# DARYL-GWZ/Proud-SLAM

Measured on AMD Instinct MI355X. Metric: rays/sec render+backward, Replica room0, 64 samples/ray, 1/2/4/8 MI355X, higher is better.
Workload: dtype f32

## Files before the change

### include/psvo.h

```cpp
#ifndef PSVO_H
#define PSVO_H

#include <stdint.h>

#ifdef __cplusplus
extern "C" {
#endif

enum {
    PSVO_OK = 0,
    PSVO_E_INVALID = 1,
    PSVO_E_LAUNCH = 2,
    PSVO_E_OVERFLOW = 3,
    PSVO_E_BUSY = 4,
    PSVO_E_SYSTEM = 5
};

const char *psvo_last_error(void);
const char *psvo_version(void);


int psvo_svo_intersect(void *stream, int b, int n, int m, float voxelsize, int n_max, const float *ray_start,
                       const float *ray_dir, const float *points, const int *children, int *idx, float *min_depth,
                       float *max_depth);
// ... 216 lines not shown

typedef struct psvo_pixel_frame {
    const float *dirs;
    const float *rgb;
    const float *depth;
    uint8_t *mask;
} psvo_pixel_frame;
int64_t psvo_sample_pixels_workspace_ints(int n_frames, int64_t n_pix);
int psvo_sample_pixels(void *stream, int n_frames, int64_t n_pix, int64_t k, const float *weights, int joint_sum,
                       const float *u, uint64_t seed, const psvo_pixel_frame *frames, int *workspace, int64_t *idx,
                       float *out_dirs, float *out_rgb, float *out_depth);

int64_t psvo_rows_workspace_ints(int64_t n_rows);
int psvo_rows_compact(void *stream, int64_t n_rows, int width, const float *grad, int *workspace, int *ids,
                      float *rows, int *count);
int psvo_rows_scatter_add(void *stream, int64_t n_list, int width, const int *ids, const float *rows, float *grad);
int psvo_rows_compact_flagged(void *stream, int64_t n_rows, int width, const float *grad, const uint8_t *flags,
                              int *workspace, int *ids, float *rows, int *count);
int psvo_rows_clear(void *stream, int64_t n_list, int width, const int *ids, float *grad, uint8_t *flags);
int psvo_rows_mark(void *stream, int64_t n_list, const int *ids, uint8_t *flags);
int psvo_rows_flags_from_grad(void *stream, int64_t n_rows, int width, const float *grad, uint8_t *flags);

psvo_engine *psvo_engine_new(void);
void psvo_engine_free(psvo_engine *e);
enum { PSVO_XCH_GATHER_I32 = 1, PSVO_XCH_SUM_I32 = 2, PSVO_XCH_SUM_F64 = 3, PSVO_XCH_QUERY = 0x100 };
typedef int (*psvo_exchange_fn)(void *user, int op, int64_t in_off, int64_t out_off, int64_t count, void *stream);
int64_t psvo_engine_exchange_words(int world, int64_t max_rays_global, int64_t max_rays_rank);
int psvo_engine_set_exchange(psvo_engine *e, int rank, int world, int64_t max_rays_global, int64_t max_rays_rank,
                             psvo_exchange_fn fn, void *user, int *xi32, double *xf64);

int psvo_engine_queued(psvo_engine *e);
int psvo_map_discard(psvo_engine *e);

enum { PSVO_PATH_QUERY_SPLIT = 1, PSVO_PATH_PADDED = 2, PSVO_PATH_DENSE_DECODER = 4 };
int psvo_engine_set_paths(psvo_engine *e, int paths);

int psvo_engine_select_stats(psvo_engine *e, void *stream, int64_t *out, int reset);

int psvo_engine_gate_stream(psvo_engine *e, void *stream);

int psvo_debug_set_lookback(int mask, int spin_bound, int delay_us);
int psvo_debug_lb_helps(int64_t *out3, int reset);
int psvo_debug_set_pixel_draw(int mode);
int psvo_debug_select_samples(void *stream, int64_t r_hit, int s_max, float truncation, float max_depth,
                              const int *offsets, const int *ray_ns, const float *z_vals, int z_stride,
                              const int *rank_ray, const float *gt_depth, const float *sdf_s, const float *feat,
                              const int *leaf, const float *t, const int *ray_of, int64_t cap, int split, int *cidx,
                              int *offa, int *offb, float *feat_c, int *leaf_c, float *t_c, int *ray_of_c,
                              float *rgb_c, int *src_c, int *counts, uint64_t *desc, uint32_t tag, int *host_flag);
int64_t psvo_debug_select_granules(int64_t r_hit);
int psvo_debug_composite_loss(void *stream, int64_t r_hit, int s_max, float truncation, float max_depth,
                              const int *offsets, const int *ray_ns, const float *z_vals, int z_stride,
                              const int *rank_ray, const float *gt_rgb, const float *gt_depth, const float *sdf_s,
                              const float *rgb_s, const float *coef, float *workspace, float *color, float *depth,
                              float *grad_sdf_s, float *grad_rgb_s, int partials, const int *cidx);

enum { PSVO_TIME_MLP_FWD = 0, PSVO_TIME_MLP_BWD = 1, PSVO_TIME_INTERP_FWD = 2, PSVO_TIME_INTERP_BWD = 3,
       PSVO_TIME_INTERSECT = 4, PSVO_TIME_SAMPLE = 5, PSVO_TIME_POINTS = 6, PSVO_TIME_SELECT = 7,
       PSVO_TIME_REGIONS = 8 };
int psvo_engine_set_timing(psvo_engine *e, int on);
int psvo_engine_timing(psvo_engine *e, double *mean_ms);
int psvo_engine_set_clock(psvo_engine *e, int max_steps);
int psvo_engine_clock(psvo_engine *e, double *period_ms, int *n_steps);
int psvo_host_wait_stats(double *wait_us, long long *calls, long long *waited, int reset);

int psvo_map_query(psvo_engine *e, void *stream, const psvo_map_desc *d, int64_t n_rays, const float *rays_o,
                   const float *rays_d, uint64_t seed);
int psvo_map_step(psvo_engine *e, void *stream, const psvo_map_desc *d, int64_t n_rays, const float *rays_o,
                  const float *rays_d, const float *gt_rgb, const float *gt_depth, uint64_t seed, int64_t adam_step,
                  int flags, float *loss_out, int *stats_out);

typedef struct psvo_map_frames {
    int n_frames;
    int64_t rays_per_frame;
    const float *dirs_cam;
    float *poses, *pose_m, *pose_v;
    const int64_t *pose_step;
    double lr_pose;
    float *pose_grad;
    const float *next_dirs_cam;
    uint64_t next_seed;
    void *next_stream;
    const float *next_gt_depth;
// ... 105 lines not shown
```

### proud-slam_amd/csrc/engine.cpp

```cpp
#include <stdio.h>
#include <stdlib.h>
#include <string.h>

#include <utility>

#include "engine_internal.h"

namespace psvo {
RenderWs *&engine_render_ws(psvo_engine *e) { return e->render; }
bool engine_data_parallel(const psvo_engine *e) { return e->x.on(); }
}

using namespace psvo;
using namespace psvo::eng;

namespace psvo {
thread_local KernelClock *g_kclock = nullptr;

namespace eng {

void *arena_buf(Arena &a, hipStream_t st, int slot, size_t bytes, int *rc) {
    if (bytes == 0) bytes = 16;
    if (a.cap[slot] >= bytes) return a.p[slot];
    if (a.p[slot]) {
// ... 189 lines not shown
    for (int i = 0; i < cnt; ++i) steps[i] = adam_step;
    for (int f = 0; pa && f < pa->n; ++f, ++cnt) {
        p[cnt] = pa->p[f];
        g[cnt] = pa->g[f];
        m[cnt] = pa->m[f];
        v[cnt] = pa->v[f];
        n[cnt] = 6;
        lr[cnt] = pa->lr;
        zero[cnt] = 0;
        steps[cnt] = pa->step[f];
    }
    return adam_launch(st, cnt, p, g, m, v, n, lr, d->beta1, d->beta2, d->eps, 0.0, adam_step, zero, steps, rows);
}

int pose_adam(hipStream_t st, const psvo_map_desc *d, const PoseAdam &pa) {
    if (pa.n == 0) return PSVO_OK;
    int64_t n6[kXchMaxFrames];
    double lr[kXchMaxFrames];
    int zero[kXchMaxFrames];
    for (int k = 0; k < pa.n; ++k) {
        n6[k] = 6;
        lr[k] = pa.lr;
        zero[k] = 0;
    }
    return adam_launch(st, pa.n, pa.p, pa.g, pa.m, pa.v, n6, lr, d->beta1, d->beta2, d->eps, 0.0, 1, zero,
                       const_cast<int64_t *>(pa.step));
}

}
}

extern "C" psvo_engine *psvo_engine_new(void) {
    psvo_engine *e = new psvo_engine();
    for (auto &q : e->qs)
        if (query_set_init(q) != PSVO_OK) {
            psvo_engine_free(e);
            return nullptr;
        }
    return e;
}

static EngineExchange exchange_layout(int world, int64_t max_rays_global, int64_t max_rays_rank) {
    EngineExchange x;
    x.world = world;
    x.nch = dist_slot0_rows(max_rays_global) / kSamplerG;
    x.max_rays_rank = max_rays_rank > 0 ? max_rays_rank : max_rays_global;
    x.cw = dist_count_words((int)x.max_rays_rank);
    return x;
}

extern "C" int64_t psvo_engine_exchange_words(int world, int64_t max_rays_global, int64_t max_rays_rank) {
    if (world < 1 || max_rays_global < 1 || max_rays_rank < 0 || max_rays_rank > max_rays_global) return -1;
    const EngineExchange x = exchange_layout(world, max_rays_global, max_rays_rank);
    return x.table_off() + x.table_words();
}

extern "C" int psvo_engine_set_exchange(psvo_engine *e, int rank, int world, int64_t max_rays_global,
                                        int64_t max_rays_rank, psvo_exchange_fn fn, void *user, int *xi32,
                                        double *xf64) {
    PSVO_REQUIRE(e, "engine_set_exchange: null engine");
    PSVO_REQUIRE(world >= 1 && rank >= 0 && rank < world && max_rays_global >= 1 && max_rays_rank >= 0 &&
                     max_rays_rank <= max_rays_global,
                 "engine_set_exchange: bad rank %d / world %d / max_rays_global %lld / max_rays_rank %lld", rank,
                 world, (long long)max_rays_global, (long long)max_rays_rank);
    PSVO_REQUIRE(e->q_count == 0, "engine_set_exchange: queries are queued");
    PSVO_REQUIRE(!fn || (xi32 && xf64), "engine_set_exchange: exchange buffers required");
    e->x = exchange_layout(world, max_rays_global, max_rays_rank);
    e->x.fn = fn;
    e->x.user = user;
    e->x.rank = rank;
    e->x.xi32 = xi32;
    e->x.xf64 = xf64;
    return PSVO_OK;
}

extern "C" int psvo_engine_set_paths(psvo_engine *e, int paths) {
    PSVO_REQUIRE(e && (paths & ~(PSVO_PATH_QUERY_SPLIT | PSVO_PATH_PADDED | PSVO_PATH_DENSE_DECODER)) == 0, "engine_set_paths: bad arguments");
    PSVO_REQUIRE(e->q_count == 0, "engine_set_paths: queries are queued");
    e->paths = paths;
    return PSVO_OK;
}

extern "C" int psvo_engine_gate_stream(psvo_engine *e, void *stream) {
    PSVO_REQUIRE(e, "engine_gate_stream: null engine");
    e->draw_gate_used = true;
    if (!e->draw_gate_recorded) return PSVO_OK;
    return st_wait(as_stream(stream), e->draw_gate_ev, "engine_gate_stream");
}

extern "C" int psvo_engine_select_stats(psvo_engine *e, void *stream, int64_t *out, int reset) {
    PSVO_REQUIRE(e && out, "engine_select_stats: null argument");
    for (int i = 0; i < 5; ++i) out[i] = 0;
    if (!e->a.p[kSelCnt]) return PSVO_OK;
    hipStream_t st = as_stream(stream);
    int c[psvo::kSelCountInts];
    if (hipMemcpyAsync(c, e->a.p[kSelCnt], sizeof(c), hipMemcpyDeviceToHost, st) != hipSuccess ||
        hipStreamSynchronize(st) != hipSuccess)
        return set_error(PSVO_E_LAUNCH, "engine_select_stats: copy failed");
    unsigned long long u[3];
    memcpy(u, c + 4, sizeof(u));
    out[0] = (int64_t)c[0] + c[1];
    out[1] = c[3];
    out[2] = (int64_t)u[0];
    out[3] = (int64_t)u[1];
    out[4] = (int64_t)u[2];
    if (c[2] & psvo::kLbFlagTimeout) {
        ENG_CALL(zero_async(static_cast<int *>(e->a.p[kSelCnt]) + 2, sizeof(int), st, "engine_select_stats"));
        if (e->host_flags) *(volatile int *)e->host_flags = 0;
        e->sel_zero_gen = 0;
        return set_error(PSVO_E_LAUNCH, "engine_select_stats: a sample selection's look-back wait was abandoned");
// ... 163 lines not shown
```

### proud-slam_amd/csrc/engine_step.cpp

```cpp
#include <stdint.h>
#include <string.h>

#include <algorithm>

#include "engine_internal.h"

using namespace psvo;
using namespace psvo::eng;

namespace {

struct Samples {
    int *offsets = nullptr, *leaf = nullptr, *ray_of = nullptr;
    float *tt = nullptr, *feat = nullptr, *rgb_s = nullptr, *act = nullptr;
    uint64_t *masks = nullptr;
};

struct Render {
    int64_t r_hit = 0, m = 0;
    int s_max = 0;
    int *rank_ray = nullptr, *ray_rank = nullptr, *ray_ns = nullptr;
    float *z_vals = nullptr, *images = nullptr, *sdf_s = nullptr;
    Samples s;
    float *sdf = nullptr, *weights = nullptr, *color = nullptr, *depth = nullptr;
    bool z_recorded = false;
    int z_stride = 0;
    bool sparse = false;
    float *h2 = nullptr;
};

constexpr int64_t kW128 = 128;
constexpr int kCritFlags = PSVO_CRIT_USE_COLOR | PSVO_CRIT_USE_DEPTH | PSVO_CRIT_USE_SDF;

void render_begin(QuerySet &qset, const Readback &rb, Render &o) {
    o.r_hit = rb.r_hit;
    o.m = rb.m;
    o.s_max = rb.s_max;
    o.rank_ray = static_cast<int *>(qset.a.p[kRankRay]);
// ... 98 lines not shown
        ENG_CALL(fork_join(st, e->aux, e->prep_fork));
        ENG_CALL(mlp_images(e->aux, c.d->width, c.d->dec, images));
        ENG_CALL(ev_record(e->prep_done, e->aux, c.who));
    }
    return PSVO_OK;
}

struct EarlyFwd {
    bool on = false;
    int64_t cap = 0;
    float *feat = nullptr, *sdf = nullptr, *h2 = nullptr;
};
int device_forward(const MapRender &c, const Images &im, Render &o, EarlyFwd &ef) {
    psvo_engine *e = c.e;
    hipStream_t st = c.st;
    const psvo_map_desc *d = c.d;
    QuerySet &qset = c.qset;
    int rc = PSVO_OK;
    const int64_t m_early = std::min<int64_t>(e->m_early, (int64_t)qset.R * qset.max_steps);
    ef.on = c.rays_path && c.sparse && qset.compacted && qset.a.p[kMDev] && m_early > 0 && im.ready() &&
            !(e->paths & PSVO_PATH_QUERY_SPLIT);
    if (!ef.on) return PSVO_OK;
    ef.cap = m_early;
    const int *m_dev = static_cast<const int *>(qset.a.p[kMDev]);
    ENG_BUF(float, fe, kFeat, m_early * 16 * sizeof(float));
    ENG_BUF(float, se, kSdfS, m_early * sizeof(float));
    ef.feat = fe;
    ef.sdf = se;
    if (d->width == 128) {
        ENG_BUF(float, he, kH2, m_early * kW128 * sizeof(float));
        ef.h2 = he;
    }
    ENG_CALL(join_adam(e, st, c.who, 2000.0));
    mark(e, st, PSVO_TIME_INTERP_FWD, 0);
    ENG_CALL(psvo::interp_fwd_dev(st, m_early, m_dev, d->voxel_size, static_cast<const int *>(qset.a.p[kLeafQ]),
                                  static_cast<const float *>(qset.a.p[kTQ]),
                                  static_cast<const int *>(qset.a.p[kRayOfQ]),
                                  static_cast<const int *>(qset.a.p[kRankRay]), c.rays_o, c.rays_d, d->centres,
                                  d->vertex_idx, d->emb, ef.feat));
    mark(e, st, PSVO_TIME_INTERP_FWD, 1);
    mark(e, st, PSVO_TIME_MLP_FWD, 0);
    if (im.on_aux) ENG_CALL(st_wait(st, e->prep_done, c.who));
    const psvo::H2Rows h2o{ef.h2, nullptr, nullptr};
    ENG_CALL(mlp_fwd_prepared(st, m_early, d->width, ef.feat, im.buf, ef.sdf, nullptr, nullptr, nullptr, m_dev, &h2o));
    if (engine_overlap(e) && c.need_z_event) {
        ENG_CALL(ev_record(e->z_ready, st, c.who));
        o.z_recorded = true;
    }
    return PSVO_OK;
}

int place_samples(const MapRender &c, Render &o) {
    psvo_engine *e = c.e;
    hipStream_t st = c.st;
    QuerySet &qset = c.qset;
    if (!c.rays_path) {
        ENG_CALL(padded_samples(e, st, qset, o));
        if (engine_overlap(e)) {
            ENG_CALL(ev_record(e->z_ready, st, c.who));
            o.z_recorded = true;
        }
        return PSVO_OK;
    }
    if (qset.compacted) {
        o.s.leaf = static_cast<int *>(qset.a.p[kLeafQ]);
        o.s.tt = static_cast<float *>(qset.a.p[kTQ]);
        o.s.ray_of = static_cast<int *>(qset.a.p[kRayOfQ]);
    }
    if (engine_overlap(e) && c.need_z_event && !o.z_recorded) {
        ENG_CALL(ev_record(e->z_ready, st, c.who));
        o.z_recorded = true;
    }
    if (!qset.compacted) {
        mark(e, st, PSVO_TIME_POINTS, 0);
        ENG_CALL(psvo::compact_rays(st, o.r_hit, qset.max_steps, static_cast<const int *>(qset.a.p[kSIdx]),
                                    static_cast<const float *>(qset.a.p[kSDepth]), o.s.offsets, o.s.leaf, o.s.tt,
                                    o.s.ray_of));
// ... 639 lines not shown
```

### proud-slam_amd/csrc/interp_load.h

```cpp
#pragma once

#include "psvo_common.h"

namespace psvo {

struct InterpSrc {
    const int *leaf, *ray_of, *ray_index, *vertex_idx;
    const float *t, *rays_o, *rays_d, *centres;
    const float4 *emb;
    float voxel_size;
};

int mlp_fwd_interp(hipStream_t st, int64_t m_cap, const int *m_dev, const InterpSrc &ip, const float *images,
                   float *sdf, float *rgb);

namespace iload {

__device__ __forceinline__ void load_x_interp(const InterpSrc &ip, int64_t s, bool valid, int h, float (&x)[8]) {
    float f[8];
#pragma unroll
    for (int i = 0; i < 8; ++i) f[i] = 0.0f;
    if (valid) {
        const int lf = ip.leaf[s];
        const int r = ip.ray_index[ip.ray_of[s]];
        const float ts = ip.t[s];
        float p[3];
#pragma unroll
        for (int a = 0; a < 3; ++a) {
            const float xa = __fadd_rn(ip.rays_o[(int64_t)r * 3 + a], __fmul_rn(ip.rays_d[(int64_t)r * 3 + a], ts));
            p[a] = __fadd_rn(__fdiv_rn(__fsub_rn(xa, ip.centres[(int64_t)lf * 3 + a]), ip.voxel_size), 0.5f);
        }
        const float ax[2] = {__fsub_rn(1.0f, p[0]), p[0]};
        const float ay[2] = {__fsub_rn(1.0f, p[1]), p[1]};
        const float az[2] = {__fsub_rn(1.0f, p[2]), p[2]};
        const int4 v0 = *reinterpret_cast<const int4 *>(ip.vertex_idx + (int64_t)lf * 8);
        const int4 v1 = *reinterpret_cast<const int4 *>(ip.vertex_idx + (int64_t)lf * 8 + 4);
        const int vid[8] = {v0.x, v0.y, v0.z, v0.w, v1.x, v1.y, v1.z, v1.w};
        float4 e0[8], e1[8];
#pragma unroll
        for (int k = 0; k < 8; ++k) {
            e0[k] = ip.emb[(int64_t)vid[k] * 4 + 2 * h];
            e1[k] = ip.emb[(int64_t)vid[k] * 4 + 2 * h + 1];
        }
#pragma unroll
        for (int k = 0; k < 8; ++k) {
            const float w = __fmul_rn(__fmul_rn(ax[(k >> 2) & 1], ay[(k >> 1) & 1]), az[k & 1]);
            f[0] = __fadd_rn(f[0], __fmul_rn(w, e0[k].x));
            f[1] = __fadd_rn(f[1], __fmul_rn(w, e0[k].y));
            f[2] = __fadd_rn(f[2], __fmul_rn(w, e0[k].z));
            f[3] = __fadd_rn(f[3], __fmul_rn(w, e0[k].w));
            f[4] = __fadd_rn(f[4], __fmul_rn(w, e1[k].x));
            f[5] = __fadd_rn(f[5], __fmul_rn(w, e1[k].y));
            f[6] = __fadd_rn(f[6], __fmul_rn(w, e1[k].z));
            f[7] = __fadd_rn(f[7], __fmul_rn(w, e1[k].w));
        }
    }
#pragma unroll
    for (int j = 0; j < 4; ++j) {
        const float send = h ? f[2 * j] : f[2 * j + 1];
        const float recv = __shfl_xor(send, 32, 64);
        x[j] = h ? recv : f[2 * j];
        x[4 + j] = h ? f[2 * j + 1] : recv;
    }
}

}
}
```

### proud-slam_amd/csrc/mlp.hip

```cpp
#include <hip/hip_runtime.h>

#include <cstdlib>

#include "interp_fuse.h"
#include "interp_load.h"
#include "psvo_common.h"

#ifdef PSVO_STAMPS
__device__ unsigned long long psvo_g_stamps[3][256][8][8][16];
#endif

namespace psvo {
namespace {

typedef float f32x16 __attribute__((ext_vector_type(16)));

constexpr int kW = 128;
constexpr int kIn = 16;
constexpr int kNB = kW / 32;

constexpr int kOffB1 = 0, kOffB2 = kOffB1 + 128, kOffB3 = kOffB2 + 128, kOffB4 = kOffB3 + 132,
              kOffB5 = kOffB4 + 128;
constexpr int kOffW3r0 = kOffB5 + 4, kOffW5 = kOffW3r0 + 128;
constexpr int kOffW = kOffW5 + 3 * 128;
// ... 644 lines not shown
                    const_cast<float *>(cm), 0, __builtin_amdgcn_readfirstlane((int)tbytes), 0x00020000);
#pragma unroll
                for (int r = 0; r < 16; ++r)
                    __builtin_amdgcn_raw_buffer_store_b32(__float_as_uint(bacc[3][r]), rc,
                                                          cfs.voff[((r >> 1) & 1) + 2 * ((r >> 2) & 1)],
                                                          4096 * 3 + 1024 * (r >> 2) + 128 * (r & 3), 0);
            }
        }
        ++seq;
        const uint64_t m4 = (uint64_t)half4[0] | ((uint64_t)half4[1] << 32);
        if (save_mask && valid) {
            uint64_t *mk = masks + (s * 2 + h) * 3;
            mk[0] = m1;
            mk[1] = m2;
            mk[2] = m4;
        }
        float rgb[3];
#pragma unroll
        for (int c = 0; c < 3; ++c) rgb[c] = sigmoidf(lds[kOffB5 + c] + row_dot(lds + kOffW5 + 128 * c, bacc, h));
        if (valid && h == 0) {
            sdf_out[s] = sdf;
            rgb_out[s * 3 + 0] = rgb[0];
            rgb_out[s * 3 + 1] = rgb[1];
            rgb_out[s * 3 + 2] = rgb[2];
        }
        if (!H2) PSVO_STAMP(8);
        PSVO_STAMP_FLUSH(0);
    }
    wait_vm(0);
}

constexpr int kLdsSdf2 = (kF2Buf0 + 16384) * 4;

template <bool IP = false>
__global__ __launch_bounds__(kF2Threads, 1) void k_mlp_sdf2(int64_t m_host, const float *__restrict__ feat,
                                                            const float *__restrict__ img,
                                                            float *__restrict__ sdf_out, const int *__restrict__ m_dev,
                                                            float *__restrict__ h2_out, InterpSrc ip) {
    extern __shared__ __attribute__((aligned(16))) float lds[];
    int64_t m = m_dev ? (int64_t)__builtin_amdgcn_readfirstlane(*m_dev) : m_host;
    if (m > m_host) m = 0;
    const int lane = threadIdx.x & 63;
    const int wave = threadIdx.x >> 6;
    const int h = lane >> 5;
    float *w2 = lds + kF2Buf0;
    const int64_t n_units = (m + kTileS - 1) / kTileS;
    const int64_t u0 = n_units * blockIdx.x / gridDim.x, u1 = n_units * (blockIdx.x + 1) / gridDim.x;
    float xn[8];
    {
        const int64_t s = (u0 + wave) * kTileS + (lane & 31);
        if constexpr (IP)
            iload::load_x_interp(ip, s, u0 + wave < u1 && s < m, h, xn);
        else
            load_x(feat, s, u0 + wave < u1 && s < m, h, xn);
    }
    stage8(lds, img + kImgVec, kVecPad, wave, lane);
    stage8(lds + kF2W1, img + kImgF1, 2048, wave, lane);
    stage8(w2, img + kImgF2, 16384, wave, lane);
    wait_vm(0);
    raw_barrier();
    for (int64_t u = u0 + wave; u < u1; u += kF2Waves) {
        const int64_t s = u * kTileS + (lane & 31);
        const bool valid = s < m;
        float x[8];
#pragma unroll
        for (int i = 0; i < 8; ++i) x[i] = xn[i];
        if (u + kF2Waves < u1) {
            const int64_t sn = (u + kF2Waves) * kTileS + (lane & 31);
            if constexpr (IP)
                iload::load_x_interp(ip, sn, sn < m, h, xn);
            else
                load_x(feat, sn, sn < m, h, xn);
        }
        f32x16 a[kNB], bacc[kNB];
        init_bias(a, lds + kOffB1, h);
        gemm_x(lds + kF2W1, x, a, lane);
        (void)relu(a);
        init_bias(bacc, lds + kOffB2, h);
        gemm_acc<kNB, kNB>(w2, a, bacc, lane);
        (void)relu(bacc);
        const float sdf = __fadd_rn(lds[kOffB3], row_dot(lds + kOffW3r0, bacc, h));
        if (valid && h == 0) sdf_out[s] = sdf;
        if (h2_out) store_rows(h2_out, s, valid, kW, bacc, h);
    }
    wait_vm(0);
}

constexpr int kU = 16;
constexpr int kUImg = 128 * kU;
constexpr int kB3Slot = kVecPad;
constexpr int kB3Small = kB3Slot + 2 * 4 * kUImg;
constexpr int kB3X = kB3Small + 2 * 4 * 4 * kU;
constexpr int kB3I = kB3X + 2 * 4 * 16 * kU;
constexpr int kB3A = kB3I + 4 * 512;
constexpr int kB3W5 = kB3A + 4 * 2 * 1024;
constexpr int kLdsBwd3 = (kB3W5 + 4 * 64 * 8) * 4;
static_assert(kLdsBwd3 <= 160 * 1024, "bwd3 LDS budget");

typedef float f32x4v __attribute__((ext_vector_type(4)));

__device__ __forceinline__ f32x4v mfma16(float a, float b, f32x4v c) {
    return __builtin_amdgcn_mfma_f32_16x16x4f32(a, b, c, 0, 0, 0);
// ... 1066 lines not shown
    psvo::launch(k_mlp_prep, dim3(div_up(kImgTotal, 256)), dim3(256), 0, as_stream(stream), p, images);
    return check_launch("mlp_images");
}
int mlp_fwd_prepared(void *stream, int64_t m, int width, const float *feat, float *images, float *sdf, float *rgb,
                     float *act, uint64_t *masks, const int *m_dev, const H2Rows *h2) {
    return mlp_fwd_impl(stream, m, width, feat, nullptr, images, sdf, rgb, act, masks, m_dev, h2);
}
int mlp_fwd(void *stream, int64_t m, int width, const float *feat, const float *const *dec, float *images, float *sdf,
            float *rgb, float *act, uint64_t *masks) {
    return mlp_fwd_impl(stream, m, width, feat, dec, images, sdf, rgb, act, masks);
}
int mlp_fwd_interp(hipStream_t st, int64_t m_cap, const int *m_dev, const InterpSrc &ip, const float *images,
                   float *sdf, float *rgb) {
    PSVO_REQUIRE(m_cap >= 0 && m_dev && images && sdf, "mlp_fwd_interp: bad arguments");
    if (m_cap == 0) return PSVO_OK;
    static bool attr = false;
    if (!attr) {
        (void)hipFuncSetAttribute(reinterpret_cast<const void *>(&k_mlp_sdf2<true>),
                                  hipFuncAttributeMaxDynamicSharedMemorySize, kLdsSdf2);
        (void)hipFuncSetAttribute(reinterpret_cast<const void *>(&k_mlp_fwd2<false, true>),
                                  hipFuncAttributeMaxDynamicSharedMemorySize, kLdsFwd2);
        attr = true;
    }
    const int64_t tiles = div_up(m_cap, kF2Tile);
    const int grid = (int)(tiles < device_cus() ? tiles : device_cus());
    if (rgb == nullptr)
        psvo::launch(k_mlp_sdf2<true>, dim3(grid), dim3(kF2Threads), kLdsSdf2, st, m_cap, nullptr, images, sdf, m_dev,
                     nullptr, ip);
    else
        psvo::launch(k_mlp_fwd2<false, true>, dim3(grid), dim3(kF2Threads), kLdsFwd2, st, m_cap, nullptr, images, sdf,
                     rgb, nullptr, nullptr, m_dev, nullptr, nullptr, ip);
    return check_launch("mlp_fwd_interp");
}
}

extern "C" int psvo_mlp_fwd(void *stream, int64_t m, int width, const float *feat, const float *w1, const float *b1,
                            const float *w2, const float *b2, const float *w3, const float *b3, const float *w4,
                            const float *b4, const float *w5, const float *b5, float *images, float *sdf, float *rgb,
                            float *act, uint64_t *masks) {
    const float *const dec[10] = {w1, b1, w2, b2, w3, b3, w4, b4, w5, b5};
    return mlp_fwd_impl(stream, m, width, feat, dec, images, sdf, rgb, act, masks);
}

static const int kDwRows[5] = {128, 128, 129, 128, 3};
static const int kDwCols[5] = {16, 128, 128, 144, 128};
static int bwd3_grid(int64_t m) {
    const int64_t rounds = (m + 4 * kU - 1) / (4 * kU);
    return (int)(rounds < device_cus() ? (rounds > 0 ? rounds : 1) : device_cus());
}
static void dw_grid_uniform(int n, DwGrid *g, int *slab_floats) {
    int off = 0;
    for (int l = 0; l < 5; ++l) {
        g->n_split[l] = n;
        g->slab_off[l] = off;
        g->slab_len[l] = kDwRows[l] * kDwCols[l] + kDwRows[l];
        off += n * g->slab_len[l];
    }
    *slab_floats = off;
}

extern "C" int64_t psvo_mlp_workspace_floats_w(int64_t m, int width, int n_split);

extern "C" int64_t psvo_mlp_workspace_floats(int64_t m, int n_split) {
    (void)n_split;
    DwGrid g;
    int slab;
// ... 146 lines not shown
```

### proud-slam_amd/psvo/_lib.py

```python
from __future__ import annotations

import ctypes
import os

import torch

PKG_ROOT = os.path.dirname(os.path.dirname(os.path.abspath(__file__)))
LIB_PATH = os.environ.get("PSVO_LIB_PATH") or os.path.join(PKG_ROOT, "lib", "libpsvo.so")

_vp, _i32, _i64, _f32, _f64, _u64 = (ctypes.c_void_p, ctypes.c_int, ctypes.c_int64, ctypes.c_float,
                                      ctypes.c_double, ctypes.c_uint64)

_SIGNATURES = {
    "psvo_last_error": (ctypes.c_char_p, []),
    "psvo_version": (ctypes.c_char_p, []),
    "psvo_svo_intersect": (_i32, [_vp, _i32, _i32, _i32, _f32, _i32] + [_vp] * 7),
    "psvo_inverse_cdf_sampling": (_i32, [_vp, _i32, _i32, _i32, _i32, _f32] + [_vp] * 9),
    "psvo_ball_intersect": (_i32, [_vp, _i32, _i32, _i32, _f32, _i32] + [_vp] * 6),
    "psvo_aabb_intersect": (_i32, [_vp, _i32, _i32, _i32, _f32, _i32] + [_vp] * 6),
    "psvo_triangle_intersect": (_i32, [_vp, _i32, _i32, _i32, _f32, _f32, _i32] + [_vp] * 6),
    "psvo_uniform_ray_sampling": (_i32, [_vp, _i32, _i32, _i32, _i32, _f32] + [_vp] * 7),
    "psvo_ray_intersect_sorted": (_i32, [_vp, _i64, _vp, _vp, _vp, _vp, _f32, _f32, _f32] + [_vp] * 6),
    "psvo_hit_rank": (_i32, [_vp, _i64, _vp, _vp, _vp]),
    "psvo_sample_rays": (_i32, [_vp, _i64, _i32, _vp, _vp, _vp, _vp, _vp, _f32, _vp, _u64, _vp, _vp, _vp, _vp,
# ... 23 lines not shown
    "psvo_sample_pixels": (_i32, [_vp, _i32, _i64, _i64, _vp, _i32, _vp, _u64, _vp, _vp, _vp, _vp, _vp, _vp]),
    "psvo_rows_compact": (_i32, [_vp, _i64, _i32, _vp, _vp, _vp, _vp, _vp]),
    "psvo_rows_scatter_add": (_i32, [_vp, _i64, _i32, _vp, _vp, _vp]),
    "psvo_rows_compact_flagged": (_i32, [_vp, _i64, _i32, _vp, _vp, _vp, _vp, _vp, _vp]),
    "psvo_rows_clear": (_i32, [_vp, _i64, _i32, _vp, _vp, _vp]),
    "psvo_rows_mark": (_i32, [_vp, _i64, _vp, _vp]),
    "psvo_rows_flags_from_grad": (_i32, [_vp, _i64, _i32, _vp, _vp]),
    "psvo_mlp_image_floats": (_i64, []),
    "psvo_mlp_image_floats_w": (_i64, [_i32]),
    "psvo_mlp_act_floats": (_i64, [_i64, _i32]),
    "psvo_mlp_mask_words": (_i64, [_i64, _i32]),
    "psvo_mlp_workspace_floats_w": (_i64, [_i64, _i32, _i32]),
    "psvo_map_grad_floats_w": (_i64, [_i64, _i32]),
    "psvo_mlp_fwd": (_i32, [_vp, _i64, _i32] + [_vp] * 16),
    "psvo_mlp_workspace_floats": (_i64, [_i64, _i32]),
    "psvo_mlp_bwd": (_i32, [_vp, _i64, _i32] + [_vp] * 28 + [_i32, _i32, _vp]),
    "psvo_criterion_workspace_floats": (_i64, [_i64]),
    "psvo_criterion_sums": (_i32, [_vp, _i64, _i32, _i32, _f32, _f32] + [_vp] * 9),
    "psvo_criterion_finalize": (_i32, [_vp, _vp, _i64, _i32, _f32, _f32, _f32, _f32, _f32, _i32, _vp]),
    "psvo_criterion_bwd": (_i32, [_vp, _i64, _i32, _f32, _f32] + [_vp] * 12),
    "psvo_adam_step": (_i32, [_vp, _i32, _vp, _vp, _vp, _vp, _vp, _f64, _f64, _f64, _f64, _f64, _i64]),
    "psvo_engine_new": (_vp, []),
    "psvo_engine_free": (None, [_vp]),
    "psvo_engine_set_timing": (_i32, [_vp, _i32]),
    "psvo_engine_set_paths": (_i32, [_vp, _i32]),
    "psvo_engine_select_stats": (_i32, [_vp, _vp, _vp, _i32]),
    "psvo_engine_gate_stream": (_i32, [_vp, _vp]),
    "psvo_debug_set_lookback": (_i32, [_i32, _i32, _i32]),
    "psvo_debug_set_pixel_draw": (_i32, [_i32]),
    "psvo_debug_lb_helps": (_i32, [_vp, _i32]),
    "psvo_debug_select_samples": (_i32, [_vp, _i64, _i32, _f32, _f32, _vp, _vp, _vp, _i32] + [_vp] * 7
                                  + [_i64, _i32] + [_vp] * 11 + [ctypes.c_uint32, _vp]),
    "psvo_debug_select_granules": (_i64, [_i64]),
    "psvo_debug_composite_loss": (_i32, [_vp, _i64, _i32, _f32, _f32, _vp, _vp, _vp, _i32] + [_vp] * 11
                                  + [_i32, _vp]),
    "psvo_engine_queued": (_i32, [_vp]),
    "psvo_map_discard": (_i32, [_vp]),
    "psvo_engine_exchange_words": (_i64, [_i32, _i64, _i64]),
    "psvo_engine_set_exchange": (_i32, [_vp, _i32, _i32, _i64, _i64, _vp, _vp, _vp, _vp]),
    "psvo_engine_timing": (_i32, [_vp, _vp]),
    "psvo_engine_set_clock": (_i32, [_vp, _i32]),
    "psvo_engine_clock": (_i32, [_vp, _vp, _vp]),
    "psvo_host_wait_stats": (_i32, [_vp, _vp, _vp, _i32]),
    "psvo_map_step": (_i32, [_vp, _vp, _vp, _i64, _vp, _vp, _vp, _vp, _u64, _i64, _i32, _vp, _vp]),
    "psvo_map_adam": (_i32, [_vp, _vp, _vp, _i64]),
    "psvo_map_adam_ex": (_i32, [_vp, _vp, _vp, _i64, _i32]),
    "psvo_map_join": (_i32, [_vp, _vp]),
    "psvo_map_side_wait": (_i32, [_vp, _vp]),
    "psvo_engine_grad_rays": (_i32, [_vp, _vp, _i64, _vp, _vp]),
    "psvo_map_query": (_i32, [_vp, _vp, _vp, _i64, _vp, _vp, _u64]),
    "psvo_map_step_frames": (_i32, [_vp, _vp, _vp, _vp, _vp, _vp, _vp, _u64, _i64, _i32, _vp, _vp]),
    "psvo_pose_rays_frames": (_i32, [_vp, _i64, _i64, _vp, _vp, _vp, _vp]),
    "psvo_pose_grad_frames": (_i32, [_vp, _i32, _i64, _i64, _vp, _vp, _vp, _vp, _vp, _vp]),
    "psvo_track_step": (_i32, [_vp, _vp, _vp, _i64, _vp, _vp, _vp, _vp, _vp, _vp, _f64, _vp, _u64, _i64, _i32, _vp,
                               _vp, _vp]),
    "psvo_render_frame": (_i32, [_vp, _vp, _vp, _i64, _vp, _vp, _vp, _u64, _vp, _vp, _vp, _vp, _vp, _vp]),
    "psvo_render_tile_bytes": (_i64, [_i64, _i32, _i32]),
    "psvo_pose_rays": (_i32, [_vp, _i64, _vp, _vp, _vp, _vp]),
    "psvo_mesh_linspace": (_i32, [_i32, _vp]),
    "psvo_mesh_case_table": (_i32, [_vp, _vp]),
    "psvo_mesh_grid_feat": (_i32, [_vp, _i64, _i32, _f32, _vp, _vp, _vp, _vp]),
    "psvo_mesh_point_feat": (_i32, [_vp, _i64, _f32, _vp, _vp, _vp, _vp, _vp, _vp]),
    "psvo_mesh_mc_count": (_i32, [_vp, _i64, _i32] + [_vp] * 6),
    "psvo_mesh_mc_emit": (_i32, [_vp, _i64, _i32, _f32] + [_vp] * 7),
    "psvo_mesh_vox_map_slots": (_i64, [_i64]),
    "psvo_mesh_vertex_rows": (_i32, [_vp, _i64, _vp, _i64, _vp, _f32, _vp, _vp]),
# ... 116 lines not shown
```

### proud-slam_amd/psvo/engine.py

```python
from __future__ import annotations

import ctypes
import os

import torch

from . import _lib as L

_vp, _i32, _i64, _f32, _f64 = ctypes.c_void_p, ctypes.c_int, ctypes.c_int64, ctypes.c_float, ctypes.c_double


class MapDesc(ctypes.Structure):
    _fields_ = [("n_nodes", _i64), ("centres", _vp), ("structure", _vp), ("vertex_idx", _vp),
                ("emb", _vp), ("n_emb", _i64), ("emb_m", _vp), ("emb_v", _vp),
                ("dec", _vp * 10), ("dec_m", _vp * 10), ("dec_v", _vp * 10), ("width", _i32),
                ("voxel_size", _f32), ("step_size", _f32), ("max_distance", _f32), ("truncation", _f32),
                ("max_depth", _f32), ("w_rgb", _f32), ("w_depth", _f32), ("w_fs", _f32), ("w_sdf", _f32),
                ("lr_emb", _f64), ("lr_dec", _f64), ("beta1", _f64), ("beta2", _f64), ("eps", _f64),
                ("grad_flat", _vp), ("packed", _vp), ("emb_row_flags", _vp), ("emb_row_local", _vp)]


class MapFrames(ctypes.Structure):
    _fields_ = [("n_frames", _i32), ("rays_per_frame", _i64), ("dirs_cam", _vp), ("poses", _vp), ("pose_m", _vp),
                ("pose_v", _vp), ("pose_step", _vp), ("lr_pose", _f64), ("pose_grad", _vp),
# ... 243 lines not shown
                                   ro.data_ptr(), rd.data_ptr(), int(seed))
        if rc != 0:
            raise self._error("psvo_map_query", rc)
        self._queued.append((rays_o, rays_d, int(seed), ro, rd))

    def step(self, rays_o, rays_d, rgb, depth, seed, apply_adam=True):
        if self._queued:
            q_o, q_d, q_seed, ro, rd = self._queued[0]
            if q_o is not rays_o or q_d is not rays_d or q_seed != int(seed):
                raise RuntimeError("MappingEngine.step: rays / seed differ from the batch query() queued "
                                   "(pass the same tensor objects and seed)")
        else:
            ro = rays_o.reshape(-1, 3).float().contiguous()
            rd = rays_d.reshape(-1, 3).float().contiguous()
        gt_rgb = rgb.reshape(-1, 3).float().contiguous()
        gt_d = depth.reshape(-1).float().contiguous()
        self.step_no += 1
        rc = _lib().psvo_map_step(self.handle, L.stream_of(ro.device), ctypes.addressof(self.desc), ro.shape[0],
                                  ro.data_ptr(), rd.data_ptr(), gt_rgb.data_ptr(), gt_d.data_ptr(), int(seed),
                                  self.step_no, 0 if apply_adam else 1, self.loss_out.data_ptr(),
                                  ctypes.addressof(self.stats))
        self._sync_queue()
        if rc != 0:
            self.step_no -= 1
            raise self._error("psvo_map_step", rc)
        return self.loss_out[0]

    def adam(self):
        ge = self.grad_exchange
        marked = ge is not None and ge.take_rows_marked()
        L.call("psvo_map_adam_ex", self.handle, L.stream_of(self.emb.device), ctypes.addressof(self.desc),
               self.step_no, 1 if marked else 0)

    PATH_QUERY_SPLIT, PATH_PADDED, PATH_DENSE_DECODER = 1, 2, 4

    def set_paths(self, paths):
        L.call("psvo_engine_set_paths", self.handle, int(paths))

    def select_stats(self, reset=False):
        out = (ctypes.c_int64 * 5)()
        L.call("psvo_engine_select_stats", self.handle, L.stream_of(self.emb.device), ctypes.cast(out, ctypes.c_void_p),
               int(bool(reset)))
        return {"kept": out[0], "composited": out[1], "kept_sum": out[2], "composited_sum": out[3], "steps": out[4]}

    def set_timing(self, on):
        L.call("psvo_engine_set_timing", self.handle, 2 if on == "overlap" else int(bool(on)))

    def set_clock(self, max_steps):
        L.call("psvo_engine_set_clock", self.handle, int(max_steps))

    def clock(self):
        ms, n = ctypes.c_double(), ctypes.c_int()
        L.call("psvo_engine_clock", self.handle, ctypes.byref(ms), ctypes.byref(n))
        return (ms.value if ms.value >= 0 else None), n.value

    @staticmethod
    def host_wait_stats(reset=False):
        us, calls, waited = ctypes.c_double(), ctypes.c_longlong(), ctypes.c_longlong()
        L.call("psvo_host_wait_stats", ctypes.byref(us), ctypes.byref(calls), ctypes.byref(waited), int(reset))
        return us.value, calls.value, waited.value

    REGIONS = ("mlp_fwd", "mlp_bwd", "interp_fwd", "interp_bwd", "intersect", "sample", "points", "select")

    def timing(self):
        out = (ctypes.c_double * len(self.REGIONS))()
        L.call("psvo_engine_timing", self.handle, ctypes.cast(out, ctypes.c_void_p))
        return dict(zip(self.REGIONS, list(out)))
# ... 114 lines not shown
```

Before: 6.305 million.

## Fuse trilinear feature interpolation into the MLP trunk kernel

```diff
diff --git a/include/psvo.h b/include/psvo.h
--- a/include/psvo.h
+++ b/include/psvo.h
@@ -272,7 +272,7 @@
 int psvo_engine_queued(psvo_engine *e);
 int psvo_map_discard(psvo_engine *e);
 
-enum { PSVO_PATH_QUERY_SPLIT = 1, PSVO_PATH_PADDED = 2, PSVO_PATH_DENSE_DECODER = 4 };
+enum { PSVO_PATH_QUERY_SPLIT = 1, PSVO_PATH_PADDED = 2, PSVO_PATH_DENSE_DECODER = 4, PSVO_PATH_INTERP_PASS = 8 };
 int psvo_engine_set_paths(psvo_engine *e, int paths);
 
 int psvo_engine_select_stats(psvo_engine *e, void *stream, int64_t *out, int reset);
@@ -289,6 +289,12 @@
                               int *offa, int *offb, float *feat_c, int *leaf_c, float *t_c, int *ray_of_c,
                               float *rgb_c, int *src_c, int *counts, uint64_t *desc, uint32_t tag, int *host_flag);
 int64_t psvo_debug_select_granules(int64_t r_hit);
+int psvo_debug_trunk_interp(void *stream, int fused, int64_t m_cap, const int *m_dev, const int *leaf, const float *t,
+                            const int *ray_of, const int *ray_index, const float *rays_o, const float *rays_d,
+                            const float *centres, const int *vertex_idx, const float *emb, float voxel_size,
+                            const float *w1, const float *b1, const float *w2, const float *b2, const float *w3,
+                            const float *b3, const float *w4, const float *b4, const float *w5, const float *b5,
+                            float *images, float *sdf, float *h2, float *feat);
 int psvo_debug_composite_loss(void *stream, int64_t r_hit, int s_max, float truncation, float max_depth,
                               const int *offsets, const int *ray_ns, const float *z_vals, int z_stride,
                               const int *rank_ray, const float *gt_rgb, const float *gt_depth, const float *sdf_s,
diff --git a/proud-slam_amd/csrc/engine.cpp b/proud-slam_amd/csrc/engine.cpp
--- a/proud-slam_amd/csrc/engine.cpp
+++ b/proud-slam_amd/csrc/engine.cpp
@@ -245,6 +245,8 @@
 
 extern "C" psvo_engine *psvo_engine_new(void) {
     psvo_engine *e = new psvo_engine();
+    const char *ipass = getenv("PSVO_INTERP_PASS");
+    if (ipass && ipass[0] == '1') e->paths |= PSVO_PATH_INTERP_PASS;
     for (auto &q : e->qs)
         if (query_set_init(q) != PSVO_OK) {
             psvo_engine_free(e);
@@ -288,7 +290,9 @@
 }
 
 extern "C" int psvo_engine_set_paths(psvo_engine *e, int paths) {
-    PSVO_REQUIRE(e && (paths & ~(PSVO_PATH_QUERY_SPLIT | PSVO_PATH_PADDED | PSVO_PATH_DENSE_DECODER)) == 0, "engine_set_paths: bad arguments");
+    PSVO_REQUIRE(e && (paths & ~(PSVO_PATH_QUERY_SPLIT | PSVO_PATH_PADDED | PSVO_PATH_DENSE_DECODER |
+                               PSVO_PATH_INTERP_PASS)) == 0,
+                 "engine_set_paths: bad arguments");
     PSVO_REQUIRE(e->q_count == 0, "engine_set_paths: queries are queued");
     e->paths = paths;
     return PSVO_OK;
diff --git a/proud-slam_amd/csrc/engine_step.cpp b/proud-slam_amd/csrc/engine_step.cpp
--- a/proud-slam_amd/csrc/engine_step.cpp
+++ b/proud-slam_amd/csrc/engine_step.cpp
@@ -4,6 +4,7 @@
 #include <algorithm>
 
 #include "engine_internal.h"
+#include "interp_load.h"
 
 using namespace psvo;
 using namespace psvo::eng;
@@ -168,17 +169,28 @@
         ef.h2 = he;
     }
     ENG_CALL(join_adam(e, st, c.who, 2000.0));
-    mark(e, st, PSVO_TIME_INTERP_FWD, 0);
-    ENG_CALL(psvo::interp_fwd_dev(st, m_early, m_dev, d->voxel_size, static_cast<const int *>(qset.a.p[kLeafQ]),
-                                  static_cast<const float *>(qset.a.p[kTQ]),
-                                  static_cast<const int *>(qset.a.p[kRayOfQ]),
-                                  static_cast<const int *>(qset.a.p[kRankRay]), c.rays_o, c.rays_d, d->centres,
-                                  d->vertex_idx, d->emb, ef.feat));
-    mark(e, st, PSVO_TIME_INTERP_FWD, 1);
+    const int *leaf_q = static_cast<const int *>(qset.a.p[kLeafQ]);
+    const float *t_q = static_cast<const float *>(qset.a.p[kTQ]);
+    const int *ray_of_q = static_cast<const int *>(qset.a.p[kRayOfQ]);
+    const int *rank_ray = static_cast<const int *>(qset.a.p[kRankRay]);
+    const bool fused = d->width == 128 && !(e->paths & PSVO_PATH_INTERP_PASS);
+    if (!fused) {
+        mark(e, st, PSVO_TIME_INTERP_FWD, 0);
+        ENG_CALL(psvo::interp_fwd_dev(st, m_early, m_dev, d->voxel_size, leaf_q, t_q, ray_of_q, rank_ray, c.rays_o,
+                                      c.rays_d, d->centres, d->vertex_idx, d->emb, ef.feat));
+        mark(e, st, PSVO_TIME_INTERP_FWD, 1);
+    }
     mark(e, st, PSVO_TIME_MLP_FWD, 0);
     if (im.on_aux) ENG_CALL(st_wait(st, e->prep_done, c.who));
-    const psvo::H2Rows h2o{ef.h2, nullptr, nullptr};
-    ENG_CALL(mlp_fwd_prepared(st, m_early, d->width, ef.feat, im.buf, ef.sdf, nullptr, nullptr, nullptr, m_dev, &h2o));
+    if (fused) {
+        const psvo::InterpSrc ip{leaf_q, ray_of_q, rank_ray, d->vertex_idx, t_q, c.rays_o, c.rays_d, d->centres,
+                                 reinterpret_cast<const float4 *>(d->emb), d->voxel_size};
+        ENG_CALL(psvo::mlp_trunk_interp(st, m_early, m_dev, ip, im.buf, ef.sdf, ef.h2, ef.feat));
+    } else {
+        const psvo::H2Rows h2o{ef.h2, nullptr, nullptr};
+        ENG_CALL(mlp_fwd_prepared(st, m_early, d->width, ef.feat, im.buf, ef.sdf, nullptr, nullptr, nullptr, m_dev,
+                                  &h2o));
+    }
     if (engine_overlap(e) && c.need_z_event) {
         ENG_CALL(ev_record(e->z_ready, st, c.who));
         o.z_recorded = true;
diff --git a/proud-slam_amd/csrc/interp_load.h b/proud-slam_amd/csrc/interp_load.h
--- a/proud-slam_amd/csrc/interp_load.h
+++ b/proud-slam_amd/csrc/interp_load.h
@@ -13,46 +13,58 @@
 
 int mlp_fwd_interp(hipStream_t st, int64_t m_cap, const int *m_dev, const InterpSrc &ip, const float *images,
                    float *sdf, float *rgb);
+int mlp_trunk_interp(hipStream_t st, int64_t m_cap, const int *m_dev, const InterpSrc &ip, const float *images,
+                     float *sdf, float *h2_out, float *feat_out);
 
 namespace iload {
 
-__device__ __forceinline__ void load_x_interp(const InterpSrc &ip, int64_t s, bool valid, int h, float (&x)[8]) {
+#define PSVO_ILOAD_FEAT8(ip, s, h, f)                                                                            \
+    const int lf = ip.leaf[s];                                                                                   \
+    const int r = ip.ray_index[ip.ray_of[s]];                                                                    \
+    const float ts = ip.t[s];                                                                                    \
+    float p[3];                                                                                                  \
+    _Pragma("unroll") for (int a = 0; a < 3; ++a) {                                                              \
+        const float xa = ip.rays_o[(int64_t)r * 3 + a] + ip.rays_d[(int64_t)r * 3 + a] * ts;                     \
+        p[a] = __fdiv_rn(xa - ip.centres[(int64_t)lf * 3 + a], ip.voxel_size) + 0.5f;                            \
+    }                                                                                                            \
+    const float ax[2] = {1.0f - p[0], p[0]};                                                                     \
+    const float ay[2] = {1.0f - p[1], p[1]};                                                                     \
+    const float az[2] = {1.0f - p[2], p[2]};                                                                     \
+    const int4 v0 = *reinterpret_cast<const int4 *>(ip.vertex_idx + (int64_t)lf * 8);                            \
+    const int4 v1 = *reinterpret_cast<const int4 *>(ip.vertex_idx + (int64_t)lf * 8 + 4);                        \
+    const int vid[8] = {v0.x, v0.y, v0.z, v0.w, v1.x, v1.y, v1.z, v1.w};                                         \
+    float4 e0[8], e1[8];                                                                                         \
+    _Pragma("unroll") for (int k = 0; k < 8; ++k) {                         \
+        e0[k] = ip.emb[(int64_t)vid[k] * 4 + 2 * h];                                                             \
+        e1[k] = ip.emb[(int64_t)vid[k] * 4 + 2 * h + 1];                                                         \
+    }                                                                                                            \
+    _Pragma("unroll") for (int k = 0; k < 8; ++k) {                                                              \
+        const float w = (ax[(k >> 2) & 1] * ay[(k >> 1) & 1]) * az[k & 1];                                       \
+        f[0] = f[0] + w * e0[k].x;                                                                               \
+        f[1] = f[1] + w * e0[k].y;                                                                               \
+        f[2] = f[2] + w * e0[k].z;                                                                               \
+        f[3] = f[3] + w * e0[k].w;                                                                               \
+        f[4] = f[4] + w * e1[k].x;                                                                               \
+        f[5] = f[5] + w * e1[k].y;                                                                               \
+        f[6] = f[6] + w * e1[k].z;                                                                               \
+        f[7] = f[7] + w * e1[k].w;                                                                               \
+    }
+
+template <bool STORE = false>
+__device__ __forceinline__ void load_x_interp(const InterpSrc &ip, int64_t s, bool valid, int h, float (&x)[8],
+                                              float *feat_out = nullptr) {
     float f[8];
 #pragma unroll
     for (int i = 0; i < 8; ++i) f[i] = 0.0f;
     if (valid) {
-        const int lf = ip.leaf[s];
-        const int r = ip.ray_index[ip.ray_of[s]];
-        const float ts = ip.t[s];
-        float p[3];
-#pragma unroll
-        for (int a = 0; a < 3; ++a) {
-            const float xa = __fadd_rn(ip.rays_o[(int64_t)r * 3 + a], __fmul_rn(ip.rays_d[(int64_t)r * 3 + a], ts));
-            p[a] = __fadd_rn(__fdiv_rn(__fsub_rn(xa, ip.centres[(int64_t)lf * 3 + a]), ip.voxel_size), 0.5f);
-        }
-        const float ax[2] = {__fsub_rn(1.0f, p[0]), p[0]};
-        const float ay[2] = {__fsub_rn(1.0f, p[1]), p[1]};
-        const float az[2] = {__fsub_rn(1.0f, p[2]), p[2]};
-        const int4 v0 = *reinterpret_cast<const int4 *>(ip.vertex_idx + (int64_t)lf * 8);
-        const int4 v1 = *reinterpret_cast<const int4 *>(ip.vertex_idx + (int64_t)lf * 8 + 4);
-        const int vid[8] = {v0.x, v0.y, v0.z, v0.w, v1.x, v1.y, v1.z, v1.w};
-        float4 e0[8], e1[8];
-#pragma unroll
-        for (int k = 0; k < 8; ++k) {
-            e0[k] = ip.emb[(int64_t)vid[k] * 4 + 2 * h];
-            e1[k] = ip.emb[(int64_t)vid[k] * 4 + 2 * h + 1];
-        }
-#pragma unroll
-        for (int k = 0; k < 8; ++k) {
-            const float w = __fmul_rn(__fmul_rn(ax[(k >> 2) & 1], ay[(k >> 1) & 1]), az[k & 1]);
-            f[0] = __fadd_rn(f[0], __fmul_rn(w, e0[k].x));
-            f[1] = __fadd_rn(f[1], __fmul_rn(w, e0[k].y));
-            f[2] = __fadd_rn(f[2], __fmul_rn(w, e0[k].z));
-            f[3] = __fadd_rn(f[3], __fmul_rn(w, e0[k].w));
-            f[4] = __fadd_rn(f[4], __fmul_rn(w, e1[k].x));
-            f[5] = __fadd_rn(f[5], __fmul_rn(w, e1[k].y));
-            f[6] = __fadd_rn(f[6], __fmul_rn(w, e1[k].z));
-            f[7] = __fadd_rn(f[7], __fmul_rn(w, e1[k].w));
+        if constexpr (STORE) {
+#pragma clang fp contract(off)
+            PSVO_ILOAD_FEAT8(ip, s, h, f)
+            float4 *row = reinterpret_cast<float4 *>(feat_out + s * 16 + 8 * h);
+            row[0] = make_float4(f[0], f[1], f[2], f[3]);
+            row[1] = make_float4(f[4], f[5], f[6], f[7]);
+        } else {
+            PSVO_ILOAD_FEAT8(ip, s, h, f)
         }
     }
 #pragma unroll
@@ -64,5 +76,7 @@
     }
 }
 
+#undef PSVO_ILOAD_FEAT8
+
 }
 }
diff --git a/proud-slam_amd/csrc/mlp.hip b/proud-slam_amd/csrc/mlp.hip
--- a/proud-slam_amd/csrc/mlp.hip
+++ b/proud-slam_amd/csrc/mlp.hip
@@ -700,11 +700,13 @@
 
 constexpr int kLdsSdf2 = (kF2Buf0 + 16384) * 4;
 
-template <bool IP = false>
-__global__ __launch_bounds__(kF2Threads, 1) void k_mlp_sdf2(int64_t m_host, const float *__restrict__ feat,
+template <bool IP = false, bool FS = false>
+__global__ __launch_bounds__(kF2Threads, 1) void k_mlp_sdf2(int64_t m_host,
+                                                            std::conditional_t<FS, float, const float> *__restrict__ feat,
                                                             const float *__restrict__ img,
                                                             float *__restrict__ sdf_out, const int *__restrict__ m_dev,
                                                             float *__restrict__ h2_out, InterpSrc ip) {
+    static_assert(IP || !FS, "the feature rows are stored by the interpolating operand load");
     extern __shared__ __attribute__((aligned(16))) float lds[];
     int64_t m = m_dev ? (int64_t)__builtin_amdgcn_readfirstlane(*m_dev) : m_host;
     if (m > m_host) m = 0;
@@ -717,7 +719,9 @@
     float xn[8];
     {
         const int64_t s = (u0 + wave) * kTileS + (lane & 31);
-        if constexpr (IP)
+        if constexpr (FS)
+            iload::load_x_interp<true>(ip, s, u0 + wave < u1 && s < m, h, xn, feat);
+        else if constexpr (IP)
             iload::load_x_interp(ip, s, u0 + wave < u1 && s < m, h, xn);
         else
             load_x(feat, s, u0 + wave < u1 && s < m, h, xn);
@@ -735,7 +739,9 @@
         for (int i = 0; i < 8; ++i) x[i] = xn[i];
         if (u + kF2Waves < u1) {
             const int64_t sn = (u + kF2Waves) * kTileS + (lane & 31);
-            if constexpr (IP)
+            if constexpr (FS)
+                iload::load_x_interp<true>(ip, sn, sn < m, h, xn, feat);
+            else if constexpr (IP)
                 iload::load_x_interp(ip, sn, sn < m, h, xn);
             else
                 load_x(feat, sn, sn < m, h, xn);
@@ -1868,6 +1874,50 @@
                      rgb, nullptr, nullptr, m_dev, nullptr, nullptr, ip);
     return check_launch("mlp_fwd_interp");
 }
+int mlp_trunk_interp(hipStream_t st, int64_t m_cap, const int *m_dev, const InterpSrc &ip, const float *images,
+                     float *sdf, float *h2_out, float *feat_out) {
+    PSVO_REQUIRE(m_cap >= 0 && m_dev && images && sdf && h2_out && feat_out && ip.leaf && ip.t && ip.ray_of &&
+                     ip.ray_index && ip.voxel_size > 0.f,
+                 "mlp_trunk_interp: bad arguments");
+    PSVO_REQUIRE(m_cap <= kMaxSamples, "mlp_trunk_interp: m_cap = %lld > %lld", (long long)m_cap,
+                 (long long)kMaxSamples);
+    if (m_cap == 0) return PSVO_OK;
+    static bool attr = false;
+    if (!attr) {
+        (void)hipFuncSetAttribute(reinterpret_cast<const void *>(&k_mlp_sdf2<true, true>),
+                                  hipFuncAttributeMaxDynamicSharedMemorySize, kLdsSdf2);
+        attr = true;
+    }
+    const int64_t tiles = div_up(m_cap, kF2Tile);
+    const int grid = (int)(tiles < device_cus() ? tiles : device_cus());
+    psvo::launch(k_mlp_sdf2<true, true>, dim3(grid), dim3(kF2Threads), kLdsSdf2, st, m_cap, feat_out, images, sdf,
+                 m_dev, h2_out, ip);
+    return check_launch("mlp_trunk_interp");
+}
+}
+
+extern "C" int psvo_debug_trunk_interp(void *stream, int fused, int64_t m_cap, const int *m_dev, const int *leaf,
+                                       const float *t, const int *ray_of, const int *ray_index, const float *rays_o,
+                                       const float *rays_d, const float *centres, const int *vertex_idx,
+                                       const float *emb, float voxel_size, const float *w1, const float *b1,
+                                       const float *w2, const float *b2, const float *w3, const float *b3,
+                                       const float *w4, const float *b4, const float *w5, const float *b5,
+                                       float *images, float *sdf, float *h2, float *feat) {
+    PSVO_REQUIRE(m_dev && images && sdf && h2 && feat, "debug_trunk_interp: null argument");
+    hipStream_t st = as_stream(stream);
+    const float *const dec[10] = {w1, b1, w2, b2, w3, b3, w4, b4, w5, b5};
+    int rc = psvo::mlp_images(stream, kW, dec, images);
+    if (rc) return rc;
+    if (fused) {
+        const InterpSrc ip{leaf, ray_of, ray_index, vertex_idx, t, rays_o, rays_d, centres,
+                           reinterpret_cast<const float4 *>(emb), voxel_size};
+        return psvo::mlp_trunk_interp(st, m_cap, m_dev, ip, images, sdf, h2, feat);
+    }
+    rc = psvo::interp_fwd_dev(st, m_cap, m_dev, voxel_size, leaf, t, ray_of, ray_index, rays_o, rays_d, centres,
+                              vertex_idx, emb, feat);
+    if (rc) return rc;
+    const H2Rows h2o{h2, nullptr, nullptr};
+    return psvo::mlp_fwd_prepared(stream, m_cap, kW, feat, images, sdf, nullptr, nullptr, nullptr, m_dev, &h2o);
 }
 
 extern "C" int psvo_mlp_fwd(void *stream, int64_t m, int width, const float *feat, const float *w1, const float *b1,
diff --git a/proud-slam_amd/psvo/_lib.py b/proud-slam_amd/psvo/_lib.py
--- a/proud-slam_amd/psvo/_lib.py
+++ b/proud-slam_amd/psvo/_lib.py
@@ -79,6 +79,7 @@
     "psvo_debug_select_samples": (_i32, [_vp, _i64, _i32, _f32, _f32, _vp, _vp, _vp, _i32] + [_vp] * 7
                                   + [_i64, _i32] + [_vp] * 11 + [ctypes.c_uint32, _vp]),
     "psvo_debug_select_granules": (_i64, [_i64]),
+    "psvo_debug_trunk_interp": (_i32, [_vp, _i32, _i64] + [_vp] * 10 + [_f32] + [_vp] * 14),
     "psvo_debug_composite_loss": (_i32, [_vp, _i64, _i32, _f32, _f32, _vp, _vp, _vp, _i32] + [_vp] * 11
                                   + [_i32, _vp]),
     "psvo_engine_queued": (_i32, [_vp]),
diff --git a/proud-slam_amd/psvo/engine.py b/proud-slam_amd/psvo/engine.py
--- a/proud-slam_amd/psvo/engine.py
+++ b/proud-slam_amd/psvo/engine.py
@@ -299,7 +299,7 @@
         L.call("psvo_map_adam_ex", self.handle, L.stream_of(self.emb.device), ctypes.addressof(self.desc),
                self.step_no, 1 if marked else 0)
 
-    PATH_QUERY_SPLIT, PATH_PADDED, PATH_DENSE_DECODER = 1, 2, 4
+    PATH_QUERY_SPLIT, PATH_PADDED, PATH_DENSE_DECODER, PATH_INTERP_PASS = 1, 2, 4, 8
 
     def set_paths(self, paths):
         L.call("psvo_engine_set_paths", self.handle, int(paths))
```

New measurement: 6.389 million (median of 6 runs). 1.01x the previous value.
